# smoggy-P/gym-Drone2D-ActivePerception

Hardware: AMD Instinct MI355X
Metric: env-steps/sec (batched) at 10 agents, map_id=1 (higher is better)
Workload: dtype f64

## Files before the change

gym-drone2d-activeperception_amd/csrc/d2d_hip.hip:

```cpp
#include <hip/hip_runtime.h>
#include <math.h>
#include <stdint.h>
#include <stdio.h>
#include <stdlib.h>
#include <string.h>
#include <type_traits>

#if defined(__HIP_DEVICE_COMPILE__)
#define D2D_AS __attribute__((address_space(1)))
#endif
#include "../../include/d2d.h"
#include "../../include/d2d_hooks.h"
#include "../../include/d2d_stepped.h"
#include "../../include/d2d_swept.h"

#define D2D_TAN_QUAL __device__ __forceinline__
#define D2D_TAN_TBL_QUAL __device__ const
#include "d2d_tan.h"
#define D2D_LOG_QUAL __device__ __forceinline__
#define D2D_LOG_TBL_QUAL __device__ const
#define D2D_RNG_QUAL __device__ __forceinline__
#include "d2d_rng.h"

#define WAVE 64
// ... 431 lines not shown
  a.velx = a.vely = a.r2 = 0.0;
  a.u = a.p0 = a.p1 = a.p2 = 0;
  if (!light) {
    a.velx = ag[D2D_A_VX * N + kk];
    a.vely = ag[D2D_A_VY * N + kk];
    a.r2 = ag[D2D_A_R2 * N + kk];
    a.u = unitp[kk];
    a.p0 = prev[3 * kk];
    a.p1 = prev[3 * kk + 1];
    a.p2 = prev[3 * kk + 2];
  }
  if constexpr (ANY_LANE) {
    const int kl = klp[klen_on ? kk : 0];
    a.klen = klen_on ? kl : 1;
  } else {
    a.klen = 1;
    if (klen_on) a.klen = klp[kk];
  }
}

__device__ __forceinline__ void agent_apply(const d2d_cfg &c, const d2d_state &s, int e, int k, const LdsView &L, double inv_scale,
                                            bool move, bool light, const AgentIn &a) {
  const int N = c.N;
  double *__restrict__ ag = s.agents + (size_t)e * D2D_AF * N;
  const double cs = 0x1.bb67ae8584cabp-1, sn = 0x1.fffffffffffffp-2;
  double px = a.px, py = a.py;
  const double velx = a.velx, vely = a.vely, rr = a.rr;
  if (light) {
    L.ax[k] = px;
    L.ay[k] = py;
    L.ar[k] = rr;
    L.act[k] = a.act;
    L.klen[k] = a.klen;
    return;
  }
  if (move) {
    const double nx = px + velx * c.dt, ny = py + vely * c.dt;
    bool aliased = true;
    double pvx = velx, pvy = vely;
    if (__builtin_fma(vely, vely, velx * velx) <= 0x1.9000000000001p+4) {
      const double rx = __builtin_fma(cs, velx, (-sn) * vely);
      const double ry = __builtin_fma(sn, velx, cs * vely);
      pvx = rx;
      pvy = ry;
      aliased = false;
    }
    if (nx < c.scale + rr) pvx = fabs(pvx);
    else if (nx > c.W_px - c.scale - rr) pvx = -fabs(pvx);
    if (ny < c.scale + rr) pvy = fabs(pvy);
    else if (ny > c.H_px - c.scale - rr) pvy = -fabs(pvy);
    const double ux = aliased ? pvx : velx, uy = aliased ? pvy : vely;
    px = px + ux * c.dt;
    py = py + uy * c.dt;
    ag[D2D_A_PX * N + k] = px;
    ag[D2D_A_PY * N + k] = py;
    ag[D2D_A_VX * N + k] = pvx;
    ag[D2D_A_VY * N + k] = pvy;
  }
  L.ax[k] = px;
  L.ay[k] = py;
  L.ar[k] = rr;
  L.ar2[k] = a.r2;
  L.ncx[k] = cell_fast(px, c.scale, inv_scale);
  L.ncy[k] = cell_fast(py, c.scale, inv_scale);
  L.nu[k] = a.u;
  L.pcx[k] = a.p0;
  L.pcy[k] = a.p1;
  L.pu[k] = a.p2;
  L.act[k] = a.act;
  L.klen[k] = a.klen;
}

__device__ __forceinline__ void st_agents(const d2d_cfg &c, const d2d_state &s, int e, int lane, const Geom &g,
                                          const LdsView &L, double inv_scale, bool move, bool want_trk, bool light = false,
                                          int k_first = 0) {
  for (int k = k_first + lane; k < c.N; k += WAVE) {
    AgentIn a;
    agent_load(c, s, e, k, want_trk, a, light);
    agent_apply(c, s, e, k, L, inv_scale, move, light, a);
  }
}

__device__ __forceinline__ void st_agents_plain(const d2d_cfg &c, const d2d_state &s, int e, int lane, const Geom &g,
                                          const LdsView &L, double inv_scale, bool move, bool want_trk, bool light = false) {
  const int N = c.N;
  double *__restrict__ ag = s.agents + (size_t)e * D2D_AF * N;
  const int *__restrict__ prev = s.dyn_prev + (size_t)e * N * 3;
  const double cs = 0x1.bb67ae8584cabp-1, sn = 0x1.fffffffffffffp-2;
  for (int k = lane; k < N; k += WAVE) {
    double px = ag[D2D_A_PX * N + k], py = ag[D2D_A_PY * N + k];
    const double velx = ag[D2D_A_VX * N + k], vely = ag[D2D_A_VY * N + k];
    const double rr = ag[D2D_A_R * N + k];
    const unsigned char act = s.active[(size_t)e * N + k];
    if (light) {
      int kl = 1;
      if (want_trk && c.kf_enabled) kl = s.kf_len[(size_t)e * N + k];
      L.ax[k] = px;
      L.ay[k] = py;
      L.ar[k] = rr;
      L.act[k] = act;
      L.klen[k] = kl;
      continue;
    }
    const double r2 = ag[D2D_A_R2 * N + k];
    const int u = s.agent_unit[(size_t)e * N + k];
    const int p0 = prev[3 * k], p1 = prev[3 * k + 1], p2 = prev[3 * k + 2];
    int klen = 1;
    if (want_trk && c.kf_enabled) klen = s.kf_len[(size_t)e * N + k];
    if (move) {
      const double nx = px + velx * c.dt, ny = py + vely * c.dt;
      bool aliased = true;
      double pvx = velx, pvy = vely;
      if (__builtin_fma(vely, vely, velx * velx) <= 0x1.9000000000001p+4) {
        const double rx = __builtin_fma(cs, velx, (-sn) * vely);
        const double ry = __builtin_fma(sn, velx, cs * vely);
        pvx = rx;
        pvy = ry;
        aliased = false;
      }
      if (nx < c.scale + rr) pvx = fabs(pvx);
      else if (nx > c.W_px - c.scale - rr) pvx = -fabs(pvx);
      if (ny < c.scale + rr) pvy = fabs(pvy);
      else if (ny > c.H_px - c.scale - rr) pvy = -fabs(pvy);
      const double ux = aliased ? pvx : velx, uy = aliased ? pvy : vely;
      px = px + ux * c.dt;
      py = py + uy * c.dt;
      ag[D2D_A_PX * N + k] = px;
      ag[D2D_A_PY * N + k] = py;
      ag[D2D_A_VX * N + k] = pvx;
      ag[D2D_A_VY * N + k] = pvy;
    }
    L.ax[k] = px;
    L.ay[k] = py;
    L.ar[k] = rr;
    L.ar2[k] = r2;
    L.ncx[k] = cell_fast(px, c.scale, inv_scale);
    L.ncy[k] = cell_fast(py, c.scale, inv_scale);
    L.nu[k] = u;
    L.pcx[k] = p0;
    L.pcy[k] = p1;
    L.pu[k] = p2;
    L.act[k] = act;
    L.klen[k] = klen;
  }
}

__device__ __forceinline__ void kf_stage(const d2d_cfg &c, const d2d_state &s, int e, int lane, const LdsView &L) {
  const int n16 = c.N * (D2D_KF * 8 / 16);
  const char *src = (const char *)(s.kf + (size_t)e * c.N * D2D_KF);
  for (int base = 0; base < n16; base += WAVE) {
    const int idx = base + lane;
    if (idx < n16)
      __builtin_amdgcn_global_load_lds((const __attribute__((address_space(1))) void *)(src + (size_t)idx * 16),
                                       (__attribute__((address_space(3))) void *)((char *)L.kf + (size_t)base * 16), 16, 0, 0);
  }
}

__device__ __forceinline__ double positive_angle(double a) {
  const double two_pi = 0x1.921fb54442d18p+2;
  a = copysign(fmod_pos(fabs(a), two_pi, 0x1.45f306dc9c883p-3 ), a);
  if (a < 0.0) a += two_pi;
  return a;
}

template <bool CONE>
__device__ __forceinline__ int ray_cull(const d2d_cfg &c, int lane, const LdsView &L, double x0, double y0, double yaw0,
                                        int ccap) {
  const int N = c.N;
  const double ss = c.scale - 1.0;
  int ncand = 0;
  double lox = 0, loy = 0, hix = 0, hiy = 0;
  bool cone = false;
  if constexpr (CONE) {
    const double span = c.ray_dth * (double)(c.R - 1);
    const double pa = 0x1.921fb54442d18p+2 - yaw0 * 0x1.1df46a2529d39p-6;
    cone = span > 0.0 && span < 2.9 && fabs(pa) < 64.0;
    const float tlo = (float)(pa + c.ray_off0), thi = (float)(pa + c.ray_off0 + span);
    lox = (double)__cosf(tlo); loy = (double)__sinf(tlo);
    hix = (double)__cosf(thi); hiy = (double)__sinf(thi);
  }
  for (int k0 = 0; k0 < N; k0 += WAVE) {
    const int k = k0 + lane;
    bool cand = false;
    double px = 0, py = 0, r2 = 0, rr = 0;
    if (k < N) {
      px = L.ax[k];
      py = L.ay[k];
      r2 = L.ar2[k];
      rr = fabs(L.ar[k]);
      const double lim = rr + c.depth + 1.5 * ss + 2.0;
      const double dx = px - x0, dy = py - y0;
      cand = (dx * dx + dy * dy <= lim * lim);
      if constexpr (CONE) {
        const double olo = loy * dx - lox * dy, ohi = dy * hix - dx * hiy, reach = rr + 0.05;
        cand = cand && (!cone || (olo <= reach && ohi <= reach));
      }
      L.hit[k] = 0;
    }
    const unsigned long long m = __ballot(cand);
    const int slot = ncand + __popcll(m & ((1ull << lane) - 1ull));
    if (cand && slot < ccap) {
      L.cx[slot] = px;
      L.cy[slot] = py;
      L.cr2[slot] = r2;
      L.crr[slot] = rr;
      L.cidx[slot] = k;
    }
    ncand += __popcll(m);
  }
  return ncand;
}

template <typename M>
struct RayT {
  double xs, ys;
  M cmask;
};
template <typename M>
__device__ __forceinline__ int mask_first(M m) {
  if constexpr (sizeof(M) == 8) return __ffsll((long long)m) - 1;
  else return __ffs((int)m) - 1;
}

template <typename M>
// ... 318 lines not shown
    }
    return;
  }
  if (__all(small)) {
    for (int k0 = 0; k0 < N; k0 += WAVE) {
      const int k = k0 + lane, kc = min(k, N - 1);
      const bool on = k < N;
      const int ncx = L.ncx[kc], ncy = L.ncy[kc], nu = L.nu[kc];
      const unsigned int nval = on ? block_valid9(ncx, ncy, nu, W, H) : 0u;
#pragma unroll
      for (int q = 0; q < 9; ++q) {
        const int di = q / 3 - 1, dj = q % 3 - 1;
        if ((nval >> q) & 1u) {
          const int idx = (ncx + di) * H + (ncy + dj);
          g8[idx] = g8[idx] | 0x80;
        }
      }
    }
    wave_sync_lds();
    for (int k0 = 0; k0 < N; k0 += WAVE) {
      const int k = k0 + lane, kc = min(k, N - 1);
      const bool on = k < N;
      const int pcx = L.pcx[kc], pcy = L.pcy[kc], pu = L.pu[kc], ncx = L.ncx[kc], ncy = L.ncy[kc], nu = L.nu[kc];
      const unsigned int pval = on ? block_valid9(pcx, pcy, pu, W, H) : 0u, nval = on ? block_valid9(ncx, ncy, nu, W, H) : 0u;
      unsigned char pv[9], nv[9];
#pragma unroll
      for (int q = 0; q < 9; ++q) {
        const int di = q / 3 - 1, dj = q % 3 - 1;
        pv[q] = g8[min(max(pcx + di, 0), W - 1) * H + min(max(pcy + dj, 0), H - 1)];
        nv[q] = g8[min(max(ncx + di, 0), W - 1) * H + min(max(ncy + dj, 0), H - 1)];
      }
      unsigned int pclr = 0, nset = 0;
#pragma unroll
      for (int q = 0; q < 9; ++q) {
        pclr |= (pv[q] == D2D_DYNAMIC) ? (1u << q) : 0u;
        const unsigned char o = nv[q] & 0x7f;
        nset |= (o != D2D_OCCUPIED && o != D2D_DYNAMIC) ? (1u << q) : 0u;
      }
      unsigned int m = pclr & pval;
      while (m) {
        const int q = __ffs((int)m) - 1;
        m &= m - 1;
        gt[(pcx + q / 3 - 1) * H + (pcy + q % 3 - 1)] = D2D_UNOCCUPIED;
      }
      m = nset & nval;
      while (m) {
        const int q = __ffs((int)m) - 1;
        m &= m - 1;
        gt[(ncx + q / 3 - 1) * H + (ncy + q % 3 - 1)] = D2D_DYNAMIC;
      }
      if (on) {
        if (pcx != ncx) prev[3 * k] = ncx;
        if (pcy != ncy) prev[3 * k + 1] = ncy;
        if (pu != nu) prev[3 * k + 2] = nu;
      }
    }
    return;
  }
  for (int k = lane; k < N; k += WAVE) {
    const int ncx = L.ncx[k], ncy = L.ncy[k], nu = L.nu[k];
    const int i1 = min(ncx + nu + 1, W), j1 = min(ncy + nu + 1, H);
    for (int i = max(ncx - nu, 0); i < i1; ++i)
      for (int j = max(ncy - nu, 0); j < j1; ++j) g8[i * H + j] = g8[i * H + j] | 0x80;
  }
  wave_sync_lds();
  for (int k = lane; k < N; k += WAVE) {
    const int pcx = L.pcx[k], pcy = L.pcy[k], pu = L.pu[k], ncx = L.ncx[k], ncy = L.ncy[k], nu = L.nu[k];
    const int i1 = min(pcx + pu + 1, W), j1 = min(pcy + pu + 1, H);
    for (int i = max(pcx - pu, 0); i < i1; ++i)
      for (int j = max(pcy - pu, 0); j < j1; ++j)
        if (g8[i * H + j] == D2D_DYNAMIC) gt[i * H + j] = D2D_UNOCCUPIED;
    const int i3 = min(ncx + nu + 1, W), j3 = min(ncy + nu + 1, H);
    for (int i = max(ncx - nu, 0); i < i3; ++i)
      for (int j = max(ncy - nu, 0); j < j3; ++j) {
        const unsigned char o = g8[i * H + j] & 0x7f;
        if (o != D2D_OCCUPIED && o != D2D_DYNAMIC) gt[i * H + j] = D2D_DYNAMIC;
      }
    if (pcx != ncx) prev[3 * k] = ncx;
    if (pcy != ncy) prev[3 * k + 1] = ncy;
    if (pu != nu) prev[3 * k + 2] = nu;
  }
}

__device__ __forceinline__ void obs_full(const d2d_cfg &c, const d2d_state &s, int e, int lane, const LdsView &L, int ci, int cj,
                                         const EnvRegs &r) {
  const int W = c.W, H = c.H, Lm = c.L, edge = (c.L - 1) / 2;
  const unsigned char *d8 = (const unsigned char *)L.dmt;
  unsigned char *__restrict__ ob = s.obs_local + (size_t)e * Lm * Lm;
  const int i0 = ci - edge, j0 = cj - edge;
  const int half = lane >> 5, col = lane & 31;
  const int j = j0 + col;
  const bool jok = col < Lm && j >= 0 && j < H;
  const int jc = min(max(j, 0), H - 1);
  for (int t = 0; 2 * t < Lm; ++t) {
    const int rr = 2 * t + half, i = i0 + rr;
    const unsigned char v = d8[min(max(i, 0), W - 1) * H + jc];
    if (rr < Lm && col < Lm) ob[rr * Lm + col] = (jok && i >= 0 && i < W) ? v : (unsigned char)0;
  }
  for (int c0 = 32; c0 < Lm; ++c0) {
    const int i = i0 + lane, jj = j0 + c0;
    const unsigned char v = d8[min(max(i, 0), W - 1) * H + min(max(jj, 0), H - 1)];
    if (lane < Lm) ob[lane * Lm + c0] = (i >= 0 && i < W && jj >= 0 && jj < H) ? v : (unsigned char)0;
  }
  if (lane == 0) s.obs_yaw[e] = (float)r.yaw;
}

template <typename P>
__device__ __forceinline__ void rng_wave_regen(P key, int lane) {
  for (int i0 = 0; i0 < D2D_RNG_KEY; i0 += WAVE) {
    const int i = i0 + lane;
    uint32_t v = 0;
    if (i < D2D_RNG_KEY) {
      const int i1 = i + 1 == D2D_RNG_KEY ? 0 : i + 1;
      const int im = i + D2D_RNG_M >= D2D_RNG_KEY ? i + D2D_RNG_M - D2D_RNG_KEY : i + D2D_RNG_M;
      v = d2d_rng_twist(key[i], key[i1], key[im]);
    }
    asm volatile("s_waitcnt vmcnt(0)" ::: "memory");
    __builtin_amdgcn_wave_barrier();
    if (i < D2D_RNG_KEY) key[i] = v;
    wave_sync_global();
  }
}

__device__ __forceinline__ int nth_set_bit(unsigned long long m, int n) {
  int p = 0;
#pragma unroll
  for (int w = 32; w > 0; w >>= 1) {
    const int cnt = __popcll((m >> p) & ((1ull << w) - 1ull));
    if (n >= cnt) {
      n -= cnt;
      p += w;
    }
  }
  return p;
}

template <typename P, typename F>
__device__ __forceinline__ int rng_wave_pairs(P key, int &pos, int &regen, int cap, int m, int lane, F &&emit) {
  int got = 0;
  while (got < m) {
    if (pos >= D2D_RNG_KEY) {
      if (regen >= cap) break;
      rng_wave_regen(key, lane);
      pos = 0;
      regen += 1;
    }
    const int n = min((D2D_RNG_KEY - pos) >> 2, WAVE);
    bool ok = false;
    double v0 = 0.0, v1 = 0.0;
    if (lane < n) {
      const int w = pos + 4 * lane;
      ok = d2d_rng_attempt(d2d_rng_temper(key[w]), d2d_rng_temper(key[w + 1]), d2d_rng_temper(key[w + 2]),
                           d2d_rng_temper(key[w + 3]), &v0, &v1) != 0;
    }
    const unsigned long long am = __ballot(ok);
    const int rank = __popcll(am & ((1ull << lane) - 1ull)), na = __popcll(am), need = m - got;
    if (ok && rank < need) emit(got + rank, v0, v1);
    if (na >= need) {
      pos += 4 * (nth_set_bit(am, need - 1) + 1);
      got = m;
    } else {
      pos += 4 * n;
      got += na;
    }
  }
  return got;
// ... 279 lines not shown
    }
  }
  r.bufn += wave_sum(arch_n);
  r.bufts += wave_sum(arch_ts);
}

__device__ __forceinline__ void st_collide(const d2d_cfg &c, const d2d_state &s, int e, int lane, const LdsView &L,
                                           bool probe_wall, EnvRegs &r) {
  const int N = c.N;
  const double R = c.drone_radius;
  int col = __any(probe_wall) ? 1 : 0;
  if (!col) {
    bool dyn = false;
    for (int k = lane; k < N; k += WAVE) {
      const double dx = L.ax[k] - r.x, dy = L.ay[k] - r.y, t = L.ar[k] + R;
      const double d2 = __builtin_fma(dy, dy, dx * dx), t2 = t * t;
      bool hit = d2 < t2 && t > 0.0;
      if (fabs(d2 - t2) <= 1e-14 * t2) hit = sqrt(d2) < t;
      dyn = dyn || hit;
    }
    if (__any(dyn)) col = 2;
  }
  int dead = 0, frz = 0;
  if (col == 0) {
    const double gx = r.x - r.tx, gy = r.y - r.ty;
    if (__builtin_fma(gy, gy, gx * gx) <= 0x1.9000000000001p+6) r.sm = D2D_SM_GOAL_REACHED;
    dead = (r.fail >= 10 && __builtin_fma(r.vy, r.vy, r.vx * r.vx) == 0.0) ? 1 : 0;
    frz = ((double)r.steps >= c.max_steps && !dead) ? 1 : 0;
  }
  const int done = (col != 0) || dead || frz || (r.sm == D2D_SM_GOAL_REACHED && r.tnext >= r.ntgt);
  if (done && c.kf_enabled) {
    int an = 0, ats = 0;
    for (int k = lane; k < N; k += WAVE) {
      if (L.act[k] != 0) {
        an += 1;
        ats += L.klen[k];
      }
    }
    r.bufn += wave_sum(an);
    r.bufts += wave_sum(ats);
  }
  if (lane == 0) {
    unsigned char *f = s.flags + (size_t)e * 4;
    f[D2D_F_COLLISION] = (unsigned char)col;
    f[D2D_F_DEADLOCK] = (unsigned char)dead;
    f[D2D_F_FREEZING] = (unsigned char)frz;
    f[D2D_F_DONE] = (unsigned char)done;
  }
  r.done = done;
}

__device__ __forceinline__ void st_obs(const d2d_cfg &c, const d2d_state &s, int e, int lane, const LdsView &L,
                                       const EnvRegs &r) {
  const int n = c.L * c.L;
  unsigned char *__restrict__ ob = s.obs_local + (size_t)e * n;
  const unsigned char *dmt = (const unsigned char *)L.dmt;
  for (int idx = lane; idx < n; idx += WAVE) ob[idx] = dmt[idx];
  if (lane == 0) s.obs_yaw[e] = (float)r.yaw;
}

__device__ __forceinline__ void load_regs(const d2d_state &s, int e, EnvRegs &r) {
  const double *d = s.drone + (size_t)e * D2D_DF;
  r.x = d[D2D_D_X]; r.y = d[D2D_D_Y]; r.yaw = d[D2D_D_YAW];
  r.vx = d[D2D_D_VX]; r.vy = d[D2D_D_VY]; r.ax = d[D2D_D_AX]; r.ay = d[D2D_D_AY];
  r.tx = s.target[(size_t)e * 2]; r.ty = s.target[(size_t)e * 2 + 1];
  const int *cn = s.counters + (size_t)e * D2D_CF;
  r.steps = cn[D2D_C_STEPS]; r.fail = cn[D2D_C_FAIL]; r.sm = cn[D2D_C_SM]; r.tnext = cn[D2D_C_TGT_NEXT];
  r.ntgt = cn[D2D_C_NTGT]; r.tracked = cn[D2D_C_TRACKED]; r.bufn = cn[D2D_C_BUF_N]; r.bufts = cn[D2D_C_BUF_TS];
}

__device__ __forceinline__ void store_regs(const d2d_state &s, int e, const EnvRegs &r) {
  double *d = s.drone + (size_t)e * D2D_DF;
  d[D2D_D_X] = r.x; d[D2D_D_Y] = r.y; d[D2D_D_YAW] = r.yaw;
  d[D2D_D_VX] = r.vx; d[D2D_D_VY] = r.vy; d[D2D_D_AX] = r.ax; d[D2D_D_AY] = r.ay;
  s.target[(size_t)e * 2] = r.tx; s.target[(size_t)e * 2 + 1] = r.ty;
  int *cn = s.counters + (size_t)e * D2D_CF;
  cn[D2D_C_STEPS] = r.steps; cn[D2D_C_FAIL] = r.fail; cn[D2D_C_SM] = r.sm; cn[D2D_C_TGT_NEXT] = r.tnext;
  cn[D2D_C_TRACKED] = r.tracked; cn[D2D_C_BUF_N] = r.bufn; cn[D2D_C_BUF_TS] = r.bufts;
}

template <bool FULL, bool WIDE, bool CONE, bool TILED = false>
__device__ __forceinline__ void run_env(const d2d_cfg &c, const d2d_state &s, int e, int lane, uint32_t stages,
                                        const Geom &g, const LdsView &L, double action, EnvRegs &r, size_t noise_off = 0,
                                        bool load_r = false, const StepIn *given = nullptr, bool late_obs = false) {
  using RayMask = std::conditional_t<WIDE, unsigned long long, unsigned int>;
  const int N = c.N, W = c.W, H = c.H;
  const double inv_scale = 1.0 / c.scale;
  const bool do_ray = stages & D2D_ST_RAYCAST, do_dyn = stages & D2D_ST_DYNGRID, do_trk = stages & D2D_ST_TRACKER;
  const bool do_col = stages & D2D_ST_COLLIDE, do_obs = stages & D2D_ST_OBS, do_ctl = stages & D2D_ST_CONTROL;
  const GridIx<TILED> gx = {H, (H + 15) >> 4};
  const size_t gbytes = TILED ? (size_t)((W + 15) >> 4) * (size_t)((H + 15) >> 4) * 256 : (size_t)W * H;
  unsigned char *__restrict__ gt = s.gt + (size_t)e * gbytes;
  unsigned char *__restrict__ dm = s.dmap + (size_t)e * gbytes;

  const bool gt_staged = FULL && (do_ray || do_dyn);
  const uint32_t needs_agents = D2D_ST_AGENTS | D2D_ST_RAYCAST | D2D_ST_DYNGRID | D2D_ST_TRACKER | D2D_ST_COLLIDE;
  const bool agents_light = (stages & needs_agents) && !(stages & (D2D_ST_AGENTS | D2D_ST_RAYCAST | D2D_ST_DYNGRID));
  StepInRaw in_raw;
  AgentIn ag0;
  const bool agents_any = (stages & needs_agents) != 0;
  if (load_r) {
    in_raw.use = false;
    if (do_ctl && !given) load_inputs_raw(c, s, e, true, in_raw);
    agent_load(c, s, e, lane, do_trk || do_col, ag0, agents_light);
  }
  if constexpr (FULL) {
    if (gt_staged) grid_stage(gt, L.gtw, W * H, lane);
    if (do_obs) grid_stage(dm, L.dmt, W * H, lane);
  }
  if (load_r) {
    if (do_trk && c.kf_enabled && g.kf_lds) kf_stage(c, s, e, lane, L);
    load_regs(s, e, r);
    __builtin_amdgcn_sched_barrier(0);
  }
  StepIn in;
  if (given) {
    in = *given;
    in.action = action;
  } else if (load_r) {
    finish_inputs(in_raw, action, in);
  } else {
    load_inputs(c, s, e, action, do_ctl, in);
  }
  D2D_STAMP(1);
  if (stages & D2D_ST_FSM) st_fsm(c, s, e, r);
  const double x0 = r.x, y0 = r.y, yaw0 = r.yaw;
  if (do_ctl) st_control(c, in, r);
  D2D_STAMP(2);
  if (!load_r && do_trk && c.kf_enabled && g.kf_lds) kf_stage(c, s, e, lane, L);
  if (agents_any) {
    const bool move = (stages & D2D_ST_AGENTS) != 0;
    if (load_r) {
      if (lane < N) agent_apply(c, s, e, lane, L, inv_scale, move, agents_light, ag0);
      if (N > WAVE) st_agents(c, s, e, lane, g, L, inv_scale, move, do_trk || do_col, agents_light, WAVE);
    } else {
      st_agents_plain(c, s, e, lane, g, L, inv_scale, move, do_trk || do_col, agents_light);
    }
    if (do_trk && !do_ray)
      for (int k = lane; k < N; k += WAVE) L.hit[k] = s.hit[(size_t)e * N + k];
    wave_sync_lds();
  }
  D2D_STAMP(3);

  const int ocx = cell_fast(x0, c.scale, inv_scale), ocy = cell_fast(y0, c.scale, inv_scale);
  const int ncx_d = cell_fast(r.x, c.scale, inv_scale), ncy_d = cell_fast(r.y, c.scale, inv_scale);
  const int edge = (c.L - 1) / 2;
  const Tile wt = make_tile(ocx - g.reach, ocy - g.reach, g.ws, g.ws);
  const Tile ct = make_tile(ncx_d - edge, ncy_d - edge, c.L, c.L);
  bool probe_wall = false;
  const bool dyn_fast = do_dyn;
  DynCells dc;
  dc.pclr = dc.nfree = 0;
  if (do_col && lane < 5 && !gt_staged) {
    const double R = c.drone_radius;
    const double ox = (lane == 0) ? -R : (lane == 2 ? R : 0.0);
    const double oy = (lane == 3) ? -R : (lane == 4 ? R : 0.0);
    const double qx = r.x + ox, qy = r.y + oy;
    const bool oob = (qx >= c.W_px || qx < 0.0 || qy >= c.H_px || qy < 0.0);
    const int pi = min(max(cell_fast(qx, c.scale, inv_scale), 0), W - 1), pj = min(max(cell_fast(qy, c.scale, inv_scale), 0), H - 1);
    probe_wall = oob || gt[gx(pi, pj)] == D2D_OCCUPIED;
  }
  if constexpr (!FULL) {
    if (do_ray && do_obs && wt.cols <= 32 && wt.rows <= 24 && ct.cols <= 33 && ct.rows <= 34) {
      tile_rows2(gx, wt, (unsigned char *)L.gtw, gt, W, H, lane, (unsigned char)D2D_OCCUPIED,
                 ct, (unsigned char *)L.dmt, dm, (unsigned char)0);
    } else {
      if (do_ray) tile_load<9>(gx, wt, (unsigned char *)L.gtw, gt, W, H, lane, (unsigned char)D2D_OCCUPIED);
      if (do_obs) tile_load<9>(gx, ct, (unsigned char *)L.dmt, dm, W, H, lane, (unsigned char)0);
    }
    if (do_dyn) dyn_bitmap(c, lane, g, L);
    if (dyn_fast && lane < N) {
      if (g.dyn2p) dyn_load<true, false>(gx, c, gt, lane, L, dc);
      else dyn_load(gx, c, gt, lane, L, dc);
    }
  }

  int ncand = 0;
  if (do_ray) {
    ncand = ray_cull<CONE>(c, lane, L, x0, y0, yaw0, g.ccap);
  }
  wave_sync_lds();
  D2D_STAMP(4);
  auto landed = [&]() {
    asm volatile("s_waitcnt vmcnt(0)" ::: "memory");
    wave_sync_lds();
    if constexpr (FULL) {
      if (do_col && lane < 5 && gt_staged) {
        const double R = c.drone_radius;
        const double ox = (lane == 0) ? -R : (lane == 2 ? R : 0.0);
        const double oy = (lane == 3) ? -R : (lane == 4 ? R : 0.0);
        const double qx = r.x + ox, qy = r.y + oy;
        const bool oob = (qx >= c.W_px || qx < 0.0 || qy >= c.H_px || qy < 0.0);
        const int pi = min(max(cell_fast(qx, c.scale, inv_scale), 0), W - 1), pj = min(max(cell_fast(qy, c.scale, inv_scale), 0), H - 1);
        probe_wall = oob || ((const unsigned char *)L.gtw)[pi * H + pj] == D2D_OCCUPIED;
      }
    }
  };
  int newly = 0;
  if (do_ray) {
    bool go = false;
    for (int i0 = 0; i0 < c.R; i0 += WAVE) {
      const int i = i0 + lane;
      const RayT<RayMask> ry = ray_setup<RayMask>(c, L, i, ncand, x0, y0, yaw0);
      if (i0 == 0) {
        landed();
        D2D_STAMP(5);
        go = (0.0 < x0 && x0 < c.W_px && 0.0 < y0 && y0 < c.H_px);
        bool cover = false;
        if (ncand <= g.ccap) {
          for (int q = lane; q < ncand; q += WAVE) {
            const double dx = L.cx[q] - x0, dy = L.cy[q] - y0;
            if (go && dx * dx + dy * dy <= L.cr2[q]) {
              L.hit[L.cidx[q]] = 1;
              cover = true;
            }
          }
        } else {
          for (int k = lane; k < N; k += WAVE) {
            const double dx = L.ax[k] - x0, dy = L.ay[k] - y0;
            if (go && dx * dx + dy * dy <= L.ar2[k]) {
              L.hit[k] = 1;
              cover = true;
            }
          }
        }
        go = go && !__any(cover);
        if (go) {
          const int g0 = FULL ? ocx * H + ocy : wt.byte_index(g.reach, g.reach);
          const unsigned char w0 = ((const unsigned char *)L.gtw)[g0];
          const unsigned char v0 = (w0 == D2D_OCCUPIED) ? (unsigned char)D2D_OCCUPIED : (unsigned char)D2D_UNOCCUPIED;
          if (lane == 0) {
            dm[gx(ocx, ocy)] = v0;
            if constexpr (FULL) {
              if (do_obs) ((unsigned char *)L.dmt)[g0] = v0;
            } else {
              const unsigned int pr = (unsigned int)(ocx - ct.i0), pq = (unsigned int)(ocy - ct.j0);
              if (do_obs && pr < (unsigned int)ct.rows && pq < (unsigned int)ct.cols) ((unsigned char *)L.dmt)[pr * ct.cols + pq] = v0;
            }
          }
          go = (w0 != D2D_OCCUPIED);
        }
      }
      const bool general = ncand > (int)(8 * sizeof(RayMask)) || __any((ry.cmask & (ry.cmask - (RayMask)1)) != (RayMask)0);
      if (general) ray_march<true, FULL>(gx, c, g, L, ry, go && i < c.R, ncand, x0, y0, wt, ct, do_obs, dm);
      else ray_march<false, FULL>(gx, c, g, L, ry, go && i < c.R, ncand, x0, y0, wt, ct, do_obs, dm);
    }
    wave_sync_lds();
    D2D_STAMP(6);
    for (int k0 = 0; k0 < N; k0 += WAVE) {
      const int k = k0 + lane;
      bool nw = false;
      if (k < N) {
        const unsigned char h = L.hit[k];
        s.hit[(size_t)e * N + k] = h;
        nw = h && !L.act[k];
      }
      newly += __popcll(__ballot(nw));
    }
    if (lane == 0) s.newly[e] = newly;
    r.tracked += newly;
  } else if (FULL ? (do_obs || do_trk || do_dyn || do_col) : (do_obs || do_trk)) {
    landed();
  }
  D2D_STAMP(7);
  if (do_trk) {
    const double D2D_AS *nz = s.noise;
    if (c.sigma != 0.0 && !s.noise && s.rng) {
      st_noise_draw(c, s, e, lane, L);
      nz = s.rng_draws;
      noise_off = 0;
    }
    if (FULL && g.ncap <= 16) {
      st_tracker_elem(c, s, e, lane, g, L, r, nz, noise_off);
    } else {
      if (g.kf_lds) st_tracker_quad<true>(c, s, e, lane, g, L, r, nz, noise_off);
      else st_tracker_quad<false>(c, s, e, lane, g, L, r, nz, noise_off);
    }
  }
  D2D_STAMP(8);
  if (do_dyn) {
    if constexpr (FULL) {
      dyn_full(c, s, e, lane, L, gt);
    } else if (g.dyn2p) {
      if (lane < N) dyn_apply<1>(gx, c, s, e, lane, g, L, gt, dc);
      for (int k = WAVE + lane; k < N; k += WAVE) {
        DynCells dk;
        dyn_load<true, false>(gx, c, gt, k, L, dk);
        dyn_apply<1>(gx, c, s, e, k, g, L, gt, dk);
      }
      wave_sync_global();
      for (int k = lane; k < N; k += WAVE) {
        DynCells dk;
        dyn_load<false, true>(gx, c, gt, k, L, dk);
        dyn_apply<2>(gx, c, s, e, k, g, L, gt, dk);
      }
    } else {
      if (lane < N) dyn_apply<0>(gx, c, s, e, lane, g, L, gt, dc);
      for (int k = WAVE + lane; k < N; k += WAVE) {
        DynCells dk;
        dyn_load(gx, c, gt, k, L, dk);
        dyn_apply<0>(gx, c, s, e, k, g, L, gt, dk);
      }
    }
  }
  D2D_STAMP(9);
  if (do_col) st_collide(c, s, e, lane, L, probe_wall, r);
  D2D_STAMP(10);
  D2D_STAMP(11);
  if (do_obs) {
    wave_sync_lds();
    if constexpr (FULL) obs_full(c, s, e, lane, L, ncx_d, ncy_d, r);
    else st_obs(c, s, e, lane, L, r);
  } else if (late_obs && __builtin_amdgcn_readfirstlane(r.done)) {
    wave_sync_global();
    if constexpr (FULL) grid_stage(dm, L.dmt, W * H, lane);
    else tile_load<9>(gx, ct, (unsigned char *)L.dmt, dm, W, H, lane, (unsigned char)0);
    asm volatile("s_waitcnt vmcnt(0)" ::: "memory");
    wave_sync_lds();
    if constexpr (FULL) obs_full(c, s, e, lane, L, ncx_d, ncy_d, r);
    else st_obs(c, s, e, lane, L, r);
  }
  D2D_STAMP(12);
}

#include "d2d_plan_spec.h"
__host__ __device__ constexpr bool spec_full(int spec) { return spec == 1 || spec == 2; }
__host__ __device__ constexpr bool spec_wide(int spec) { return spec == 3 || spec == 0 || spec == 4; }
__host__ __device__ constexpr bool spec_tiled(int spec) { return spec == 4; }
__host__ __device__ constexpr bool spec_generic(int spec) { return spec == 0 || spec == 4; }
__host__ __device__ constexpr bool spec_cone(int spec) { return spec != 1; }
extern __shared__ __attribute__((aligned(16))) char d2d_lds[];

struct StagesKArgs {
  d2d_cfg c;
  d2d_state s;
  uint32_t stages;
  const double *pin;
  unsigned char *coll_out;
};

template <int SPEC>
__global__ __launch_bounds__(WAVE *WAVES_PER_BLOCK, D2D_MIN_WAVES) void k_stages(StagesKArgs args) {
#if defined(__HIP_DEVICE_COMPILE__)
  const StagesKArgs *ka = (const StagesKArgs *)(const __attribute__((address_space(4))) StagesKArgs *)__builtin_amdgcn_kernarg_segment_ptr();
#else
  const StagesKArgs *ka = nullptr;
#endif
  const d2d_cfg &c_in = args.c;
  const d2d_state &s_in = args.s;
  const uint32_t stages = args.stages;
  const double *pin = args.pin;
  unsigned char *coll_out = args.coll_out;
  d2d_cfg c_folded;
  if (!spec_generic(SPEC)) {
    c_folded = c_in;
    spec_default_apply(c_folded);
  }
  const d2d_cfg &c = !spec_generic(SPEC) ? c_folded : ka->c;
  const d2d_state &s = (SPEC == 1 || SPEC == 2) ? s_in : ka->s;
  const int lane = threadIdx.x & (WAVE - 1), wpb = (SPEC == 1 || SPEC == 2) ? WAVES_PER_BLOCK : (int)(blockDim.x / WAVE);
  const int wv = __builtin_amdgcn_readfirstlane(threadIdx.x / WAVE);
  const int e = blockIdx.x * wpb + wv;
  if (e >= c.B) return;
  if ((stages & D2D_ST_SKIP_DONE) && s.flags[(size_t)e * 4 + D2D_F_DONE] != 0) return;
  const Geom g = make_geom(c, wpb, spec_ncap(SPEC), spec_full(SPEC));
// ... 127 lines not shown
}

template <int SPEC>
__host__ __device__ inline int closed_wave_bytes(const d2d_cfg &c, const d2d_plan &p, int wpb) {
  int b = make_geom(c, wpb, spec_ncap(SPEC), spec_full(SPEC)).wave_bytes;
  const int pb = plan_wave_bytes(c.N, p.nu, p.n_sample, c.W, c.H), gb = p.gaze == D2D_GAZE_OXFORD ? gaze_geom(c, p).wave_bytes : 0;
  b = b > pb ? b : pb;
  b = b > gb ? b : gb;
  return (b + 15) & ~15;
}


#if defined(__HIP_DEVICE_COMPILE__)
typedef const ClosedArgs __attribute__((address_space(4))) *ArgsPtr;
#else
typedef const ClosedArgs *ArgsPtr;
#endif

struct PhaseIn {
  ArgsPtr a;
  int e, off, lane;
};
__device__ __forceinline__ PhaseIn phase_enter(const ClosedArgs *ap, int e_, int lds_off_) {
  const unsigned long long v = (unsigned long long)ap;
  unsigned int lo = __builtin_amdgcn_readfirstlane((unsigned int)v), hi = __builtin_amdgcn_readfirstlane((unsigned int)(v >> 32));
  int e = __builtin_amdgcn_readfirstlane(e_), off = __builtin_amdgcn_readfirstlane(lds_off_);
  int lane = threadIdx.x & (WAVE - 1);
  asm volatile("; phase" : "+s"(lo), "+s"(hi), "+s"(e), "+s"(off), "+v"(lane));
  PhaseIn in;
  in.a = (ArgsPtr)(((unsigned long long)hi << 32) | lo);
  in.e = e;
  in.off = off;
  in.lane = lane;
  return in;
}
template <bool PDEF, typename F>
__device__ __forceinline__ auto with_plan(ArgsPtr a, F f) {
  if constexpr (PDEF) {
    d2d_plan p = a->p;
    plan_default_apply(p);
    return f(p);
  } else {
    return f(a->p);
  }
}


template <int SPEC, bool PDEF>
__device__ __forceinline__ int ph_plan_quick(const ClosedArgs *ap, int e_, int lds_off_) {
  const PhaseIn in_ = phase_enter(ap, e_, lds_off_);
  const ArgsPtr a = in_.a;
  const int e = in_.e, lane = in_.lane;
  char *base = d2d_lds + in_.off;
  d2d_cfg c = a->c;
  if (!spec_generic(SPEC)) spec_default_apply(c);
  if constexpr (SPEC == 1 || SPEC == 2) {
    constexpr int cap = spec_ncap(SPEC);
    __builtin_assume(c.N <= cap);
  }
  const bool need = with_plan<PDEF>(a, [&](const d2d_plan &p) __attribute__((always_inline)) { return plan_env_quick(c, a->s, p, e, lane, base); });
  wave_sync_global();
  return need ? 1 : 0;
}

template <int SPEC, bool PDEF>
__device__ __forceinline__ void ph_plan_search(const ClosedArgs *ap, int e_, int lds_off_) {
  const PhaseIn in_ = phase_enter(ap, e_, lds_off_);
  const ArgsPtr a = in_.a;
  const int e = in_.e, lane = in_.lane;
  char *base = d2d_lds + in_.off;
  d2d_cfg c = a->c;
  if (!spec_generic(SPEC)) spec_default_apply(c);
  if constexpr (SPEC == 1 || SPEC == 2) {
    constexpr int cap = spec_ncap(SPEC);
    __builtin_assume(c.N <= cap);
  }
  with_plan<PDEF>(a, [&](const d2d_plan &p) __attribute__((always_inline)) { plan_env_search<PDEF>(c, a->s, p, e, lane, base); });
  wave_sync_global();
}

__host__ __device__ constexpr uint32_t hidden_stages(uint32_t stages) { return stages & ~(uint32_t)D2D_ST_OBS; }
__host__ __device__ constexpr bool late_obs_of(uint32_t stages) { return (stages & D2D_ST_COLLIDE) && !(stages & D2D_ST_OBS); }

template <int SPEC, bool PDEF, uint32_t ACT = D2D_ST_ACT>
__device__ __forceinline__ int ph_plan_act(const ClosedArgs *ap, int e_, int lds_off_, int &walls_ok) {
  const PhaseIn in_ = phase_enter(ap, e_, lds_off_);
  const ArgsPtr a = in_.a;
  const int e = in_.e, lane = in_.lane;
  char *base = d2d_lds + in_.off;
  d2d_cfg c = a->c;
  if (!spec_generic(SPEC)) spec_default_apply(c);
  if constexpr (SPEC == 1 || SPEC == 2) {
    constexpr int cap = spec_ncap(SPEC);
    __builtin_assume(c.N <= cap);
  }
  double4 w_head;
  int wk = __builtin_amdgcn_readfirstlane(walls_ok);
  asm volatile("; phase" : "+s"(wk));
  const bool need = with_plan<PDEF>(a, [&](const d2d_plan &p) __attribute__((always_inline)) { return plan_env_quick(c, a->s, p, e, lane, base, &w_head, &wk); });
  walls_ok = __builtin_amdgcn_readfirstlane(wk);
  if (need) {
    wave_sync_global();
    return -1;
  }
  wave_sync_lds();
  StepIn in;
  in.action = 0.0;
  in.ok = true;
  in.has_wp = true;
  in.wp[0] = w_head.x; in.wp[1] = w_head.y; in.wp[2] = w_head.z; in.wp[3] = w_head.w; in.wp[4] = 0.0; in.wp[5] = 0.0;
  const int wpb = (int)(blockDim.x / WAVE);
  const Geom g = make_geom(c, wpb, spec_ncap(SPEC), spec_full(SPEC));
  const LdsView L = carve(base, g, c.L);
  EnvRegs r;
  run_env<spec_full(SPEC), spec_wide(SPEC), spec_cone(SPEC), spec_tiled(SPEC)>(c, a->s, e, lane, ACT, g, L, a->s.action[e], r, 0, true, &in, late_obs_of(ACT));
  if (lane == 0) store_regs(a->s, e, r);
  wave_sync_global();
  return r.done;
}

template <int SPEC, bool PDEF, uint32_t STAGES>
__device__ __forceinline__ int ph_gaze_stages(const ClosedArgs *ap, int e_, int lds_off_, int t_, int done_) {
  const PhaseIn in_ = phase_enter(ap, e_, lds_off_);
  const ArgsPtr a = in_.a;
  const int e = in_.e, lane = in_.lane;
  int tstep = __builtin_amdgcn_readfirstlane(t_), known_done = __builtin_amdgcn_readfirstlane(done_);
  asm volatile("; phase" : "+s"(tstep), "+s"(known_done));
  char *base = d2d_lds + in_.off;
  d2d_cfg c = a->c;
  if (!spec_generic(SPEC)) spec_default_apply(c);
#ifdef D2D_CHAIN_PROF
  const unsigned long long pp0 = __builtin_amdgcn_s_memtime();
#endif
  with_plan<PDEF>(a, [&](const d2d_plan &p) __attribute__((always_inline)) {
    gaze_env<true, PDEF>(c, a->s, p, a->init, a->on_done == D2D_DONE_RESET, e, lane, base, known_done);
  });
  wave_sync_global();
#ifdef D2D_CHAIN_PROF
  D2D_PHASE_ADD(0, pp0);
  const unsigned long long pp1 = __builtin_amdgcn_s_memtime();
#endif
  const int wpb = (int)(blockDim.x / WAVE);
  const Geom g = make_geom(c, wpb, spec_ncap(SPEC), spec_full(SPEC));
  const LdsView L = carve(base, g, c.L);
  EnvRegs r;
  load_regs(a->s, e, r);
  const size_t noise_off = c.noise_rows > 1 ? (size_t)((c.noise_row0 + tstep) % c.noise_rows) * c.B * c.N * 2 : 0;
  run_env<spec_full(SPEC), spec_wide(SPEC), spec_cone(SPEC), spec_tiled(SPEC)>(c, a->s, e, lane, STAGES, g, L, a->s.action[e], r, noise_off, false, nullptr, late_obs_of(STAGES));
  if (lane == 0) store_regs(a->s, e, r);
  wave_sync_global();
#ifdef D2D_CHAIN_PROF
  D2D_PHASE_ADD(1, pp1);
#endif
  return r.done;
}

template <int SPEC, uint32_t STAGES>
__device__ __forceinline__ int ph_stages(const ClosedArgs *ap, int e_, int lds_off_) {
  const PhaseIn in_ = phase_enter(ap, e_, lds_off_);
  const ArgsPtr a = in_.a;
  const int e = in_.e, lane = in_.lane;
  char *base = d2d_lds + in_.off;
  d2d_cfg c = a->c;
  if (!spec_generic(SPEC)) spec_default_apply(c);
  const int wpb = (int)(blockDim.x / WAVE);
  const Geom g = make_geom(c, wpb, spec_ncap(SPEC), spec_full(SPEC));
  const LdsView L = carve(base, g, c.L);
  EnvRegs r;
  run_env<spec_full(SPEC), spec_wide(SPEC), spec_cone(SPEC), spec_tiled(SPEC)>(c, a->s, e, lane, STAGES, g, L, a->s.action[e], r, 0, true, nullptr, late_obs_of(STAGES));
  if (lane == 0) store_regs(a->s, e, r);
  wave_sync_global();
  return r.done;
}

template <int SPEC, bool PDEF = false>
__global__ __launch_bounds__(WAVE *WAVES_PER_BLOCK, D2D_MIN_WAVES) void k_closed(const ClosedArgs *__restrict__ a) {
  static_assert(!PDEF || SPEC == 1, "the plan's defaults are folded into the few-agent kernel of the default geometry only");
  const int wv = __builtin_amdgcn_readfirstlane(threadIdx.x / WAVE);
  const int wpb = (int)(blockDim.x / WAVE);
  const int e = blockIdx.x * wpb + wv;
  if (e >= a->c.B) return;
  d2d_cfg c = a->c;
  if (!spec_generic(SPEC)) spec_default_apply(c);
  int off;
  bool split;
  if constexpr (PDEF) {
    d2d_plan p = a->p;
    plan_default_apply(p);
    off = wv * closed_wave_bytes<SPEC>(c, p, wpb);
    split = p.planner == D2D_PLAN_PRIMITIVE;
  } else {
    off = wv * closed_wave_bytes<SPEC>(c, a->p, wpb);
    split = a->p.planner == D2D_PLAN_PRIMITIVE;
  }
  const int nsteps = a->nsteps;
  const bool freeze = a->on_done == D2D_DONE_FREEZE;
  const bool obs_every = a->obs_every != 0;
  int nsearch = 0;
  int walls_ok = 0;
#ifdef D2D_CHAIN_PROF
  const unsigned long long cp0 = __builtin_amdgcn_s_memtime();
  unsigned long long cps = 0;
#endif
  int flag_done = a->s.flags[(size_t)e * 4 + D2D_F_DONE] != 0 ? 1 : 0;
#pragma unroll 1
  for (int t = 0; t < nsteps; ++t) {
    if (freeze && flag_done != 0) break;
    const bool visible = obs_every || t == nsteps - 1;
    if (split) {
      if (nsearch * 32 > t + 16) __builtin_amdgcn_s_setprio(2); else __builtin_amdgcn_s_setprio(0);
      ph_gaze_stages<SPEC, PDEF, D2D_ST_PERCEIVE>(a, e, off, t, flag_done);
#ifdef D2D_CHAIN_PROF
      const unsigned long long q0 = __builtin_amdgcn_s_memtime();
#endif
      const int pa = __builtin_amdgcn_readfirstlane(visible ? ph_plan_act<SPEC, PDEF, D2D_ST_ACT>(a, e, off, walls_ok)
                                                            : ph_plan_act<SPEC, PDEF, hidden_stages(D2D_ST_ACT)>(a, e, off, walls_ok));
#ifdef D2D_CHAIN_PROF
      D2D_PHASE_ADD(2, q0);
#endif
      if (pa < 0) {
#ifdef D2D_CHAIN_PROF
        const unsigned long long s0 = __builtin_amdgcn_s_memtime();
#endif
        ph_plan_search<SPEC, PDEF>(a, e, off);
        nsearch += 1;
        walls_ok = 0;
#ifdef D2D_CHAIN_PROF
        cps += __builtin_amdgcn_s_memtime() - s0;
        D2D_PHASE_ADD(3, s0);
        const unsigned long long a0 = __builtin_amdgcn_s_memtime();
#endif
        flag_done = __builtin_amdgcn_readfirstlane(visible ? ph_stages<SPEC, D2D_ST_ACT>(a, e, off)
                                                           : ph_stages<SPEC, hidden_stages(D2D_ST_ACT)>(a, e, off));
#ifdef D2D_CHAIN_PROF
        D2D_PHASE_ADD(4, a0);
#endif
      } else {
        flag_done = pa;
      }
    } else {
      flag_done = __builtin_amdgcn_readfirstlane(visible ? ph_gaze_stages<SPEC, PDEF, D2D_ST_ALL>(a, e, off, t, flag_done)
                                                         : ph_gaze_stages<SPEC, PDEF, hidden_stages(D2D_ST_ALL)>(a, e, off, t, flag_done));
    }
  }
#ifdef D2D_CHAIN_PROF
  if ((threadIdx.x & (WAVE - 1)) == 0 && a->p.plan_stat) {
    const unsigned long long tot = __builtin_amdgcn_s_memtime() - cp0;
    a->p.plan_stat[(size_t)e * 4 + 1] = (int)(tot >> 4);
    a->p.plan_stat[(size_t)e * 4 + 2] = (int)(cps >> 4);
  }
#endif
}

#include "d2d_swept.h"

thread_local char g_err[256] = "";

int fail(int code, const char *msg) {
  snprintf(g_err, sizeof g_err, "%s", msg);
  return code;
}

constexpr size_t LDS_SOFT = 64 * 1024, LDS_HARD = 160 * 1024;

template <typename K>
void lds_optin(K kernel, size_t bytes) {
  if (bytes > LDS_SOFT) (void)hipFuncSetAttribute((const void *)kernel, hipFuncAttributeMaxDynamicSharedMemorySize, (int)bytes);
}

int launched() {
  const hipError_t err = hipGetLastError();
  return err == hipSuccess ? 0 : fail(-3, hipGetErrorString(err));
}

dim3 env_grid(int B, int wpb = WAVES_PER_BLOCK) { return dim3((B + wpb - 1) / wpb); }
dim3 env_block(int wpb = WAVES_PER_BLOCK) { return dim3(WAVE * wpb); }

int spec_of(const d2d_cfg &c) {
  if (!spec_default_matches(c)) return c.grid_tile ? 4 : 0;
  return c.N <= spec_ncap(1) ? 1 : (c.N <= spec_ncap(2) ? 2 : 3);
}

[[maybe_unused]] const void *const kInstantiationOrder[] = {
    (const void *)k_stages<3>, (const void *)k_stages<1>, (const void *)k_stages<2>, (const void *)k_stages<4>, (const void *)k_stages<0>,
    (const void *)k_closed<0>, (const void *)k_closed<4>, (const void *)k_closed<3>, (const void *)k_closed<1>, (const void *)k_closed<2>,
    (const void *)k_closed<1, true>};

template <typename F>
auto with_spec(int spec, F f) {
  switch (spec) {
    case 1: return f(IntC<1>{});
    case 2: return f(IntC<2>{});
    case 3: return f(IntC<3>{});
    case 4: return f(IntC<4>{});
    default: return f(IntC<0>{});
  }
}

template <typename F>
int best_wpb(F bytes) {
  int best = 0, best_waves = 0;
  for (int wpb = WAVES_PER_BLOCK; wpb >= 1; wpb >>= 1) {
    const size_t wg = (size_t)bytes(wpb) * wpb;
    if (wg == 0 || wg > (wpb == 1 ? LDS_HARD : LDS_SOFT)) continue;
    int waves = (int)(LDS_HARD / ((wg + 1023) & ~(size_t)1023)) * wpb;
    if (waves > 16) waves = 16;
    if (waves > best_waves) {
      best = wpb;
      best_waves = waves;
    }
  }
  return best;
}

int fit_wpb(size_t wave_bytes) {
  int wpb = WAVES_PER_BLOCK;
  while (wpb > 1 && wave_bytes * wpb > LDS_SOFT) wpb >>= 1;
  return wpb;
}

struct Launch {
  int spec;
  int wpb;
  size_t wave_bytes;
  size_t lds() const { return wave_bytes * wpb; }
// ... 362 lines not shown
```

Before: 99.34 million.

## Gate dynamic-grid updates on hidden steps after verifying grid invariant

Adds a one-time check per run (re-armed after auto-reset) that verifies the grid contains only free/dynamic-tagged cells around prior agent footprints. When the check passes, the dynamic-obstacle grid rewrite and the per-agent prev-cell loads are skipped on steps whose observation is not visible. The aim is to avoid the per-step dyn_full grid sweep when the grid state is not consumed. This adds a full-grid scan and extra gating state threaded through the phase functions, and risks stale dynamic cells if downstream stages such as raycast or collision read them.

```diff
diff --git a/gym-drone2d-activeperception_amd/csrc/d2d_hip.hip b/gym-drone2d-activeperception_amd/csrc/d2d_hip.hip
--- a/gym-drone2d-activeperception_amd/csrc/d2d_hip.hip
+++ b/gym-drone2d-activeperception_amd/csrc/d2d_hip.hip
@@ -537,7 +537,8 @@
 }
 
 __device__ __forceinline__ void st_agents_plain(const d2d_cfg &c, const d2d_state &s, int e, int lane, const Geom &g,
-                                          const LdsView &L, double inv_scale, bool move, bool want_trk, bool light = false) {
+                                          const LdsView &L, double inv_scale, bool move, bool want_trk, bool light = false,
+                                          bool dyn_feed = true) {
   const int N = c.N;
   double *__restrict__ ag = s.agents + (size_t)e * D2D_AF * N;
   const int *__restrict__ prev = s.dyn_prev + (size_t)e * N * 3;
@@ -558,8 +559,13 @@
       continue;
     }
     const double r2 = ag[D2D_A_R2 * N + k];
-    const int u = s.agent_unit[(size_t)e * N + k];
-    const int p0 = prev[3 * k], p1 = prev[3 * k + 1], p2 = prev[3 * k + 2];
+    int u = 0, p0 = 0, p1 = 0, p2 = 0;
+    if (dyn_feed) {
+      u = s.agent_unit[(size_t)e * N + k];
+      p0 = prev[3 * k];
+      p1 = prev[3 * k + 1];
+      p2 = prev[3 * k + 2];
+    }
     int klen = 1;
     if (want_trk && c.kf_enabled) klen = s.kf_len[(size_t)e * N + k];
     if (move) {
@@ -589,12 +595,14 @@
     L.ay[k] = py;
     L.ar[k] = rr;
     L.ar2[k] = r2;
-    L.ncx[k] = cell_fast(px, c.scale, inv_scale);
-    L.ncy[k] = cell_fast(py, c.scale, inv_scale);
-    L.nu[k] = u;
-    L.pcx[k] = p0;
-    L.pcy[k] = p1;
-    L.pu[k] = p2;
+    if (dyn_feed) {
+      L.ncx[k] = cell_fast(px, c.scale, inv_scale);
+      L.ncy[k] = cell_fast(py, c.scale, inv_scale);
+      L.nu[k] = u;
+      L.pcx[k] = p0;
+      L.pcy[k] = p1;
+      L.pu[k] = p2;
+    }
     L.act[k] = act;
     L.klen[k] = klen;
   }
@@ -1079,6 +1087,31 @@
   }
 }
 
+__device__ __forceinline__ bool dyn_gate_full(const d2d_cfg &c, int lane, const LdsView &L) {
+  const int N = c.N, W = c.W, H = c.H;
+  unsigned char *g8 = (unsigned char *)L.gtw;
+  for (int k = lane; k < N; k += WAVE) {
+    const int pcx = L.pcx[k], pcy = L.pcy[k], pu = L.pu[k];
+    const int i1 = min(pcx + pu + 1, W), j1 = min(pcy + pu + 1, H);
+    for (int i = max(pcx - pu, 0); i < i1; ++i)
+      for (int j = max(pcy - pu, 0); j < j1; ++j) g8[i * H + j] = g8[i * H + j] | 0x80;
+  }
+  wave_sync_lds();
+  bool bad = false;
+  const int nd = (W * H) >> 2;
+  for (int i = lane; i < nd; i += WAVE) {
+    const unsigned int w = L.gtw[i];
+#pragma unroll
+    for (int b = 0; b < 4; ++b) {
+      const unsigned int v = (w >> (8 * b)) & 0xffu;
+      bad = bad || !(((v & 0x7fu) - 1u < 2u) || v == (0x80u | D2D_DYNAMIC));
+    }
+    if (w & 0x80808080u) L.gtw[i] = w & 0x7f7f7f7fu;
+  }
+  wave_sync_lds();
+  return !__any(bad);
+}
+
 __device__ __forceinline__ void obs_full(const d2d_cfg &c, const d2d_state &s, int e, int lane, const LdsView &L, int ci, int cj,
                                          const EnvRegs &r) {
   const int W = c.W, H = c.H, Lm = c.L, edge = (c.L - 1) / 2;
@@ -1524,11 +1557,12 @@
 template <bool FULL, bool WIDE, bool CONE, bool TILED = false>
 __device__ __forceinline__ void run_env(const d2d_cfg &c, const d2d_state &s, int e, int lane, uint32_t stages,
                                         const Geom &g, const LdsView &L, double action, EnvRegs &r, size_t noise_off = 0,
-                                        bool load_r = false, const StepIn *given = nullptr, bool late_obs = false) {
+                                        bool load_r = false, const StepIn *given = nullptr, bool late_obs = false,
+                                        int *dyn_gate = nullptr, bool dyn_visible = true, bool dyn_skip = false) {
   using RayMask = std::conditional_t<WIDE, unsigned long long, unsigned int>;
   const int N = c.N, W = c.W, H = c.H;
   const double inv_scale = 1.0 / c.scale;
-  const bool do_ray = stages & D2D_ST_RAYCAST, do_dyn = stages & D2D_ST_DYNGRID, do_trk = stages & D2D_ST_TRACKER;
+  const bool do_ray = stages & D2D_ST_RAYCAST, do_dyn = (stages & D2D_ST_DYNGRID) && !dyn_skip, do_trk = stages & D2D_ST_TRACKER;
   const bool do_col = stages & D2D_ST_COLLIDE, do_obs = stages & D2D_ST_OBS, do_ctl = stages & D2D_ST_CONTROL;
   const GridIx<TILED> gx = {H, (H + 15) >> 4};
   const size_t gbytes = TILED ? (size_t)((W + 15) >> 4) * (size_t)((H + 15) >> 4) * 256 : (size_t)W * H;
@@ -1576,7 +1610,7 @@
       if (lane < N) agent_apply(c, s, e, lane, L, inv_scale, move, agents_light, ag0);
       if (N > WAVE) st_agents(c, s, e, lane, g, L, inv_scale, move, do_trk || do_col, agents_light, WAVE);
     } else {
-      st_agents_plain(c, s, e, lane, g, L, inv_scale, move, do_trk || do_col, agents_light);
+      st_agents_plain(c, s, e, lane, g, L, inv_scale, move, do_trk || do_col, agents_light, do_dyn || !dyn_gate);
     }
     if (do_trk && !do_ray)
       for (int k = lane; k < N; k += WAVE) L.hit[k] = s.hit[(size_t)e * N + k];
@@ -1722,7 +1756,14 @@
   D2D_STAMP(8);
   if (do_dyn) {
     if constexpr (FULL) {
-      dyn_full(c, s, e, lane, L, gt);
+      bool run = true;
+      if (dyn_gate) {
+        int gs = __builtin_amdgcn_readfirstlane(*dyn_gate);
+        if (gs == 0) gs = dyn_gate_full(c, lane, L) ? 1 : 2;
+        *dyn_gate = gs;
+        run = dyn_visible || gs == 2;
+      }
+      if (run) dyn_full(c, s, e, lane, L, gt);
     } else if (g.dyn2p) {
       if (lane < N) dyn_apply<1>(gx, c, s, e, lane, g, L, gt, dc);
       for (int k = WAVE + lane; k < N; k += WAVE) {
@@ -2016,6 +2057,7 @@
 __host__ __device__ constexpr uint32_t hidden_stages(uint32_t stages) { return stages & ~(uint32_t)D2D_ST_OBS; }
 __host__ __device__ constexpr bool late_obs_of(uint32_t stages) { return (stages & D2D_ST_COLLIDE) && !(stages & D2D_ST_OBS); }
 
+
 template <int SPEC, bool PDEF, uint32_t ACT = D2D_ST_ACT>
 __device__ __forceinline__ int ph_plan_act(const ClosedArgs *ap, int e_, int lds_off_, int &walls_ok) {
   const PhaseIn in_ = phase_enter(ap, e_, lds_off_);
@@ -2054,12 +2096,18 @@
 }
 
 template <int SPEC, bool PDEF, uint32_t STAGES>
-__device__ __forceinline__ int ph_gaze_stages(const ClosedArgs *ap, int e_, int lds_off_, int t_, int done_) {
+__device__ __forceinline__ int ph_gaze_stages(const ClosedArgs *ap, int e_, int lds_off_, int t_, int done_, int &dyn_gate, bool dyn_vis_) {
   const PhaseIn in_ = phase_enter(ap, e_, lds_off_);
   const ArgsPtr a = in_.a;
   const int e = in_.e, lane = in_.lane;
   int tstep = __builtin_amdgcn_readfirstlane(t_), known_done = __builtin_amdgcn_readfirstlane(done_);
   asm volatile("; phase" : "+s"(tstep), "+s"(known_done));
+  int dgate = 2;
+  const int dvis = dyn_vis_ ? 1 : 0;
+  if constexpr (spec_full(SPEC)) {
+    dgate = __builtin_amdgcn_readfirstlane(dyn_gate);
+    asm volatile("; phase" : "+s"(dgate));
+  }
   char *base = d2d_lds + in_.off;
   d2d_cfg c = a->c;
   if (!spec_generic(SPEC)) spec_default_apply(c);
@@ -2080,7 +2128,12 @@
   EnvRegs r;
   load_regs(a->s, e, r);
   const size_t noise_off = c.noise_rows > 1 ? (size_t)((c.noise_row0 + tstep) % c.noise_rows) * c.B * c.N * 2 : 0;
-  run_env<spec_full(SPEC), spec_wide(SPEC), spec_cone(SPEC), spec_tiled(SPEC)>(c, a->s, e, lane, STAGES, g, L, a->s.action[e], r, noise_off, false, nullptr, late_obs_of(STAGES));
+  if constexpr (spec_full(SPEC)) {
+    run_env<true, spec_wide(SPEC), spec_cone(SPEC), spec_tiled(SPEC)>(c, a->s, e, lane, STAGES, g, L, a->s.action[e], r, noise_off, false, nullptr, late_obs_of(STAGES), &dgate, dvis != 0, dgate == 1 && dvis == 0);
+    dyn_gate = __builtin_amdgcn_readfirstlane(dgate);
+  } else {
+    run_env<spec_full(SPEC), spec_wide(SPEC), spec_cone(SPEC), spec_tiled(SPEC)>(c, a->s, e, lane, STAGES, g, L, a->s.action[e], r, noise_off, false, nullptr, late_obs_of(STAGES));
+  }
   if (lane == 0) store_regs(a->s, e, r);
   wave_sync_global();
 #ifdef D2D_CHAIN_PROF
@@ -2130,6 +2183,8 @@
   const int nsteps = a->nsteps;
   const bool freeze = a->on_done == D2D_DONE_FREEZE;
   const bool obs_every = a->obs_every != 0;
+  const bool dyn_defer = spec_full(SPEC) && !obs_every && !freeze, auto_reset = a->on_done == D2D_DONE_RESET;
+  int dyn_gate = dyn_defer ? 0 : 2;
   int nsearch = 0;
   int walls_ok = 0;
 #ifdef D2D_CHAIN_PROF
@@ -2141,9 +2196,10 @@
   for (int t = 0; t < nsteps; ++t) {
     if (freeze && flag_done != 0) break;
     const bool visible = obs_every || t == nsteps - 1;
+    if (dyn_defer && auto_reset && flag_done != 0) dyn_gate = 0;
     if (split) {
       if (nsearch * 32 > t + 16) __builtin_amdgcn_s_setprio(2); else __builtin_amdgcn_s_setprio(0);
-      ph_gaze_stages<SPEC, PDEF, D2D_ST_PERCEIVE>(a, e, off, t, flag_done);
+      ph_gaze_stages<SPEC, PDEF, D2D_ST_PERCEIVE>(a, e, off, t, flag_done, dyn_gate, visible);
 #ifdef D2D_CHAIN_PROF
       const unsigned long long q0 = __builtin_amdgcn_s_memtime();
 #endif
@@ -2173,8 +2229,8 @@
         flag_done = pa;
       }
     } else {
-      flag_done = __builtin_amdgcn_readfirstlane(visible ? ph_gaze_stages<SPEC, PDEF, D2D_ST_ALL>(a, e, off, t, flag_done)
-                                                         : ph_gaze_stages<SPEC, PDEF, hidden_stages(D2D_ST_ALL)>(a, e, off, t, flag_done));
+      flag_done = __builtin_amdgcn_readfirstlane(visible ? ph_gaze_stages<SPEC, PDEF, D2D_ST_ALL>(a, e, off, t, flag_done, dyn_gate, true)
+                                                         : ph_gaze_stages<SPEC, PDEF, hidden_stages(D2D_ST_ALL)>(a, e, off, t, flag_done, dyn_gate, false));
     }
   }
 #ifdef D2D_CHAIN_PROF
```

After: 103.6 million, median of 6. +4.2%, better.
